# tenpy/cyten

Hardware: AMD Instinct MI355X
Metric: block-sparse tdot+SVD GFLOP/s (fp64) (higher is better)
Workload: dtype f64

## Files before the change

cyten_amd/csrc/jacobi_engine.hip:

```cpp
#include "jacobi_engine.h"

#include <algorithm>
#include <cmath>
#include <cstdlib>

namespace cyb {
constexpr double kPredictQuad = 16.0;
namespace {

typedef double d4 __attribute__((ext_vector_type(4)));
typedef double d2 __attribute__((ext_vector_type(2)));
#define GLOBAL_AS __attribute__((address_space(1)))
typedef const GLOBAL_AS d2* gc2;
typedef const GLOBAL_AS d2* gcp2;
typedef GLOBAL_AS double* gp;

constexpr int GS = JP + 2;
constexpr int QS = JP + 16;
constexpr int GK = 64;
constexpr int XS = GK + 2;
constexpr int NT = 256;
constexpr int NPAIR = JP / 2;
static_assert(JP == 32, "the wave tiling below assumes 32 x 32 pair problems");

// ... 844 lines not shown
            for (int e = lane; e < (CJ / 2) * CJ * 2; e += 64) {
                const int which = e / ((CJ / 2) * CJ), f = e % ((CJ / 2) * CJ);
                const int k = f / CJ, row = f % CJ;
                int p, q;
                pair_of(r, k, p, q);
                double* Xr = which ? Ur : Hr;
                double* Xi = which ? Ui : Hi;
                const double c = rot[k * 4], sn = rot[k * 4 + 1], fr = rot[k * 4 + 2], fi = -rot[k * 4 + 3];
                const double pr_ = Xr[row * CS + p], pi_ = Xi[row * CS + p], qr_ = Xr[row * CS + q], qi_ = Xi[row * CS + q];
                const double tr = fr * qr_ - fi * qi_, ti = fr * qi_ + fi * qr_;
                Xr[row * CS + p] = c * pr_ - sn * tr;
                Xi[row * CS + p] = c * pi_ - sn * ti;
                Xr[row * CS + q] = sn * pr_ + c * tr;
                Xi[row * CS + q] = sn * pi_ + c * ti;
            }
            __builtin_amdgcn_fence(__ATOMIC_RELEASE, "wavefront");
            __builtin_amdgcn_wave_barrier();
        }
    for (int e = lane; e < CJ * CJ; e += 64) {
        const int a = e / CJ, b = e % CJ;
        const double x = Ur[a * CS + b], y = Ui[a * CS + b];
        Vout[(2 * a) * VS + 2 * b] = x;
        Vout[(2 * a) * VS + 2 * b + 1] = -y;
        Vout[(2 * a + 1) * VS + 2 * b] = y;
        Vout[(2 * a + 1) * VS + 2 * b + 1] = x;
    }
    if (lane < CJ) {
        const double lam = Hr[lane * CS + lane];
        Gdiag[(2 * lane) * GS + 2 * lane] = lam;
        Gdiag[(2 * lane + 1) * GS + 2 * lane + 1] = lam;
    }
}

struct SScratch {
    double* gpart;
    unsigned int* ticket;
    unsigned int* ready;
    unsigned int* err;
    const int2* wgmap;
    const int2* wgent;
    unsigned long long* stamps;
    int stamp_round;
    int n_sweeps, n_mats;
    unsigned int* arrive;
    int* nsw;
    unsigned int* readyJ;
    int defer_j;
    int cross_every, cross_min_nb;
};
constexpr int SW_MAX_ENT = 64;

constexpr int SW_UN = 8;
constexpr int SW_PRE = 6;
constexpr int SWEEP_XREG = (4 * JP * GS > JP * GS + 2 * JP * VS) ? 4 * JP * GS : JP * GS + 2 * JP * VS;
constexpr int SWEEP_LDS_DOUBLES = JP * GS + SWEEP_XREG + 2 * JP * QS + 8;
constexpr size_t SWEEP_LDS_BYTES = 88 * 1024;
static_assert((size_t)SWEEP_LDS_DOUBLES * 8 + 1024 <= SWEEP_LDS_BYTES, "LDS request of the sweep kernel");
constexpr int SWEEP_WG_PER_CU = 1;

typedef unsigned int u32x2 __attribute__((ext_vector_type(2)));
union Q8 {
    u32x2 u;
    double d;
};

template <int SLEEP = 1>
__device__ __forceinline__ bool spin_until(const unsigned int* word, unsigned int target, unsigned int* err)
{
    const unsigned long long t0 = wall_clock64();
    unsigned int it = 0;
    while (__hip_atomic_load(word, __ATOMIC_RELAXED, __HIP_MEMORY_SCOPE_AGENT) < target) {
        __builtin_amdgcn_s_sleep(SLEEP);
        if ((++it & 63u) == 0u) {
            if (__hip_atomic_load(err, __ATOMIC_RELAXED, __HIP_MEMORY_SCOPE_AGENT) != 0u) return false;
            if (wall_clock64() - t0 > 100000000ull) {
                __hip_atomic_store(err, 1u, __ATOMIC_RELAXED, __HIP_MEMORY_SCOPE_AGENT);
                return false;
            }
        }
    }
    return true;
}

__device__ __forceinline__ void sweep_update_j(const __amdgpu_buffer_rsrc_t rsJ, const double* Qm, int P, int Q, int nvp, int j_begin,
                                               int nJ, int wave, int lane)
{
    const int un = lane & 15, ukq = lane >> 4;
    const double* ap0 = Qm + (lane >> 4) * QS + (lane & 15);
    const double* ap1 = ap0 + 16;
    double a0[JP / 4], a1[JP / 4];
#pragma unroll
    for (int kk = 0; kk < JP / 4; ++kk) {
        a0[kk] = ap0[kk * 4 * QS];
        a1[kk] = ap1[kk * 4 * QS];
    }
    auto off_of = [&](int c, int k) { return (unsigned int)(((int64_t)xrow(k, P, Q) * nvp + (j_begin + c) * 64 + wave * 16 + un) * 8); };
    auto load = [&](double (&x)[JP / 4], int c) {
#pragma unroll
        for (int kk = 0; kk < JP / 4; ++kk) {
            Q8 q;
            q.u = __builtin_amdgcn_raw_buffer_load_b64(rsJ, off_of(c, 4 * kk + ukq), 0, 16);
            x[kk] = q.d;
        }
    };
    double xb[JP / 4], xn[JP / 4];
    if (nJ > 0) load(xb, 0);
    for (int c = 0; c < nJ; ++c) {
        if (c + 1 < nJ) load(xn, c + 1);
        d4 acc[2] = {d4{0.0, 0.0, 0.0, 0.0}, d4{0.0, 0.0, 0.0, 0.0}};
#pragma unroll
        for (int kk = 0; kk < JP / 4; ++kk) {
            acc[0] = __builtin_amdgcn_mfma_f64_16x16x4f64(a0[kk], xb[kk], acc[0], 0, 0, 0);
            acc[1] = __builtin_amdgcn_mfma_f64_16x16x4f64(a1[kk], xb[kk], acc[1], 0, 0, 0);
        }
#pragma unroll
        for (int i = 0; i < 2; ++i)
#pragma unroll
            for (int q = 0; q < 4; ++q) {
                Q8 v;
                v.d = acc[i][q];
                __builtin_amdgcn_raw_buffer_store_b64(v.u, rsJ, off_of(c, i * 16 + (lane >> 4) + 4 * q), 0, 16);
            }
#pragma unroll
        for (int kk = 0; kk < JP / 4; ++kk) xb[kk] = xn[kk];
    }
}

template <bool CPLX>
__global__ void __launch_bounds__(NT, 1)
jacobi_sweep_kernel(const RPair* __restrict__ pairs, int max_inner, unsigned long long* __restrict__ offmax_bits, SScratch sc)
{
    extern __shared__ __attribute__((aligned(16))) double rsm[];
    double* Gs = rsm;
    double* G2 = Gs + JP * GS;
    double* Va = G2 + JP * GS;
    double* Vb = Va + JP * VS;
    double* Xc = G2;
    double* Qs0 = G2 + SWEEP_XREG;
    double* Qs1 = Qs0 + JP * QS;
    double* red = Qs1 + JP * QS;
    int* ibase = reinterpret_cast<int*>(red + 8);
    int* perm = ibase;
    int* zrow = ibase + JP;
    int* zout = ibase + 2 * JP;
    int* flags = ibase + 3 * JP;
    int* edone = flags + 4;

    const int tid = threadIdx.x;
    const int lane = tid & 63, wave = tid >> 6;
    const int2 went = sc.wgent ? sc.wgent[blockIdx.x] : make_int2((int)blockIdx.x, (int)blockIdx.x + 1);
    int max_rounds = 0;
    for (int e = went.x; e < went.y; ++e) max_rounds = max(max_rounds, pairs[sc.wgmap[e].x].nb - 1);
    const int n_sw = sc.n_sweeps;
    const bool one_entry = went.y - went.x == 1;
    int pendP = -1, pendQ = -1, pend_ground = 0;
    if (n_sw > 1) {
        if (tid < SW_MAX_ENT) edone[tid] = 0;
        __syncthreads();
    }
    for (int sw = 0; sw < n_sw; ++sw) {
    for (int round = 0; round < max_rounds; ++round)
    for (int ent = went.x; ent < went.y; ++ent) {
    const int2 wm = sc.wgmap[ent];
    const int pi = wm.x, part = wm.y;
    const RPair mt = pairs[pi];
    if (round >= mt.nb - 1) continue;
    if (n_sw > 1 && edone[ent - went.x]) continue;
    const int ground = sw * (mt.nb - 1) + round;
    const int G = mt.pad[0];
    unsigned int* ready = sc.ready + mt.pad[1];
    unsigned int* readyJ = sc.readyJ + mt.pad[1];
    unsigned int* ticket = sc.ticket + pi;
    double* Qs = (ground & 1) ? Qs1 : Qs0;
    const unsigned int pbytes = JP * JP * 8;
    const __amdgpu_buffer_rsrc_t rsW = __builtin_amdgcn_make_buffer_rsrc(mt.W, 0, (int)((size_t)mt.nvp * mt.lenp * 8), 0x00020000);
    const __amdgpu_buffer_rsrc_t rsJ =
        __builtin_amdgcn_make_buffer_rsrc(mt.J ? mt.J : mt.W, 0, mt.J ? (int)((size_t)mt.nvp * mt.nvp * 8) : 0, 0x00020000);
    const int cw = mt.lenp / 64, cj = mt.J ? mt.nvp / 64 : 0;
    const int w_begin = (int)((int64_t)part * cw / G), w_end = (int)((int64_t)(part + 1) * cw / G);
    const int j_begin = (int)((int64_t)part * cj / G), j_end = (int)((int64_t)(part + 1) * cj / G);
    const int nW = w_end - w_begin, nJ = j_end - j_begin;
    const bool defer = sc.defer_j && one_entry && G > 1 && nJ > 0 && round < mt.nb - 2;
    const int ct = defer ? nW : nW + nJ;
    const int pre_limit = (sc.defer_j && G > 1) ? min(ct, nW) : ct;
    const int un = lane & 15, ukq = lane >> 4;
#define SWEEP_STAMP(k)                                                                                            \
    do {                                                                                                          \
        if (sc.stamps && tid == 0 && round == sc.stamp_round) sc.stamps[(size_t)blockIdx.x * 8 + (k)] = wall_clock64(); \
    } while (0)

    {
        int P, Q;
        circle_pair(mt.nb, round, mt.slot, P, Q);
        if (P > Q) {
            const int t = P;
            P = Q;
            Q = t;
        }
        SWEEP_STAMP(0);
        __syncthreads();
        if (ground > 0) {
            if (tid == 0) {
                bool ok = spin_until(ready + (size_t)P * G + part, (unsigned int)ground, sc.err);
                ok = ok && spin_until(ready + (size_t)Q * G + part, (unsigned int)ground, sc.err);
                flags[1] = ok ? 1 : 0;
            }
            __syncthreads();
            if (!flags[1]) return;
        }
        SWEEP_STAMP(1);
        auto chunk_off = [&](int c, int k, bool& in_w) -> unsigned int {
            in_w = c < nW;
            const int ld = in_w ? mt.lenp : mt.nvp;
            const int cc = in_w ? w_begin + c : j_begin + (c - nW);
            return (unsigned int)(((int64_t)xrow(k, P, Q) * ld + cc * 64 + wave * 16 + un) * 8);
        };
        auto chunk_load = [&](int c, int k) -> double {
            bool in_w;
            const unsigned int off = chunk_off(c, k, in_w);
            Q8 q;
            q.u = in_w ? __builtin_amdgcn_raw_buffer_load_b64(rsW, off, 0, 16) : __builtin_amdgcn_raw_buffer_load_b64(rsJ, off, 0, 16);
            return q.d;
        };
        double xpre[SW_PRE][JP / 4];
        {
            const int ld = mt.lenp;
            d4 acc00 = d4{0.0, 0.0, 0.0, 0.0}, acc01 = acc00, acc11 = acc00;
            const int r = lane & 15, g2 = 2 * (lane >> 4);
            const unsigned int o0 = (unsigned int)(((int64_t)xrow(r, P, Q) * ld + g2) * 8);
            const unsigned int o1 = (unsigned int)(((int64_t)xrow(r + 16, P, Q) * ld + g2) * 8);
            const int c_begin = 8 * w_begin, c_end = 8 * w_end;
            constexpr int UN = SW_UN;
            d2 x0[UN], x1[UN], n0[UN], n1[UN];
            auto load = [&](d2 (&a0)[UN], d2 (&a1)[UN], int c0) {
#pragma unroll
                for (int u = 0; u < UN; ++u) {
                    const int c = min(c0 + 4 * u, c_end - 1);
                    Q16 qa, qb;
                    qa.u = __builtin_amdgcn_raw_buffer_load_b128(rsW, o0 + (unsigned int)c * 64u, 0, 16);
                    qb.u = __builtin_amdgcn_raw_buffer_load_b128(rsW, o1 + (unsigned int)c * 64u, 0, 16);
                    a0[u] = qa.d;
                    a1[u] = qb.d;
                }
            };
            if (c_begin + wave < c_end) load(x0, x1, c_begin + wave);
#pragma unroll
            for (int c = 0; c < SW_PRE; ++c) {
                if (c < pre_limit) {
#pragma unroll
                    for (int kk = 0; kk < JP / 4; ++kk) xpre[c][kk] = chunk_load(c, 4 * kk + ukq);
                }
            }
            for (int c0 = c_begin + wave; c0 < c_end; c0 += 4 * UN) {
                const bool more = c0 + 4 * UN < c_end;
                if (more) load(n0, n1, c0 + 4 * UN);
#pragma unroll
                for (int u = 0; u < UN; ++u) {
                    if (c0 + 4 * u < c_end) {
                        acc00 = __builtin_amdgcn_mfma_f64_16x16x4f64(x0[u].x, x0[u].x, acc00, 0, 0, 0);
                        acc01 = __builtin_amdgcn_mfma_f64_16x16x4f64(x0[u].x, x1[u].x, acc01, 0, 0, 0);
                        acc11 = __builtin_amdgcn_mfma_f64_16x16x4f64(x1[u].x, x1[u].x, acc11, 0, 0, 0);
                        acc00 = __builtin_amdgcn_mfma_f64_16x16x4f64(x0[u].y, x0[u].y, acc00, 0, 0, 0);
                        acc01 = __builtin_amdgcn_mfma_f64_16x16x4f64(x0[u].y, x1[u].y, acc01, 0, 0, 0);
                        acc11 = __builtin_amdgcn_mfma_f64_16x16x4f64(x1[u].y, x1[u].y, acc11, 0, 0, 0);
                    }
                }
                if (more) {
#pragma unroll
                    for (int u = 0; u < UN; ++u) {
                        x0[u] = n0[u];
                        x1[u] = n1[u];
                    }
                }
            }
            double* wpart = Xc + wave * (JP * GS);
#pragma unroll
            for (int q = 0; q < 4; ++q) {
                const int rr = (lane >> 4) + 4 * q, cc = lane & 15;
                wpart[rr * GS + cc] = acc00[q];
                wpart[rr * GS + 16 + cc] = acc01[q];
                wpart[(16 + cc) * GS + rr] = acc01[q];
                wpart[(16 + rr) * GS + 16 + cc] = acc11[q];
            }
        }
        __syncthreads();
        SWEEP_STAMP(2);
        {
            const int gi = tid >> 3, gj = 4 * (tid & 7);
            d2 lo = d2{0.0, 0.0}, hi = d2{0.0, 0.0};
#pragma unroll
            for (int w = 0; w < 4; ++w) {
                const double* src = Xc + w * (JP * GS) + gi * GS + gj;
                lo.x += src[0];
                lo.y += src[1];
                hi.x += src[2];
                hi.y += src[3];
            }
            if (G > 1) {
                const __amdgpu_buffer_rsrc_t rs_all = __builtin_amdgcn_make_buffer_rsrc(
                    sc.gpart + ((size_t)pi * 2 + (size_t)(ground & 1)) * RGMAX * (JP * JP), 0, (int)(pbytes * G), 0x00020000);
                Q16 a, b;
                a.d = lo;
                b.d = hi;
                const unsigned int off = (unsigned int)part * pbytes + (unsigned int)tid * 32u;
                __builtin_amdgcn_raw_buffer_store_b128(a.u, rs_all, off, 0, 16);
                __builtin_amdgcn_raw_buffer_store_b128(b.u, rs_all, off + 16u, 0, 16);
                asm volatile("s_waitcnt vmcnt(0)" ::: "memory");
                __syncthreads();
                if (tid == 0) __hip_atomic_fetch_add(ticket, 1u, __ATOMIC_RELAXED, __HIP_MEMORY_SCOPE_AGENT);
                if (pendP >= 0) {
                    if (tid == 0) {
                        bool ok = spin_until(readyJ + (size_t)pendP * G + part, (unsigned int)pend_ground, sc.err);
                        ok = ok && spin_until(readyJ + (size_t)pendQ * G + part, (unsigned int)pend_ground, sc.err);
                        flags[1] = ok ? 1 : 0;
                    }
                    __syncthreads();
                    if (!flags[1]) return;
                    sweep_update_j(rsJ, (pend_ground & 1) ? Qs1 : Qs0, pendP, pendQ, mt.nvp, j_begin, nJ, wave, lane);
                    asm volatile("s_waitcnt vmcnt(0)" ::: "memory");
                    __syncthreads();
                    if (tid == 0) {
                        __hip_atomic_store(readyJ + (size_t)pendP * G + part, (unsigned int)(pend_ground + 1), __ATOMIC_RELAXED, __HIP_MEMORY_SCOPE_AGENT);
                        __hip_atomic_store(readyJ + (size_t)pendQ * G + part, (unsigned int)(pend_ground + 1), __ATOMIC_RELAXED, __HIP_MEMORY_SCOPE_AGENT);
                    }
                    pendP = -1;
                }
                if (tid == 0) flags[1] = spin_until(ticket, (unsigned int)G * (unsigned int)(ground + 1), sc.err) ? 1 : 0;
                __syncthreads();
                if (!flags[1]) return;
                lo = d2{0.0, 0.0};
                hi = d2{0.0, 0.0};
                for (int g0 = 0; g0 < G; g0 += 4) {
                    Q16 pa[4], pb[4];
#pragma unroll
                    for (int g = 0; g < 4; ++g) {
                        if (g0 + g < G) {
                            pa[g].u = __builtin_amdgcn_raw_buffer_load_b128(rs_all, (unsigned int)(g0 + g) * pbytes + (unsigned int)tid * 32u, 0, 16);
                            pb[g].u = __builtin_amdgcn_raw_buffer_load_b128(rs_all, (unsigned int)(g0 + g) * pbytes + (unsigned int)tid * 32u + 16u, 0, 16);
                        }
                    }
#pragma unroll
                    for (int g = 0; g < 4; ++g) {
                        if (g0 + g < G) {
                            lo += pa[g].d;
                            hi += pb[g].d;
                        }
                    }
                }
            }
            double* dst = Gs + gi * GS + gj;
            dst[0] = lo.x;
            dst[1] = lo.y;
            dst[2] = hi.x;
            dst[3] = hi.y;
        }
        __syncthreads();
        SWEEP_STAMP(3);
        if (tid == 0) flags[0] = 0;
        __syncthreads();
        if (tid < JP) {
            double g = Gs[tid * GS + tid];
            if constexpr (CPLX) g = fmax(g, Gs[(tid ^ 1) * GS + (tid ^ 1)]);
            const int z = (g > 0.0 && g <= mt.thr2) ? 1 : 0;
            zrow[tid] = z;
            perm[tid] = tid;
            if (z) flags[0] = 1;
        }
        __syncthreads();
        const bool any_null = flags[0] != 0;
        if (any_null) {
            for (int e = tid; e < JP * JP; e += NT) {
                const int i = e / JP, j = e % JP;
                if (zrow[i] || zrow[j]) Gs[i * GS + j] = 0.0;
            }
            __syncthreads();
        }
        const double off = gram_offmax(Gs, red, tid);
        if (part == 0 && tid == 0) atomicMax(offmax_bits + (size_t)sw * sc.n_mats + mt.mat, (unsigned long long)__double_as_longlong(off));
        const bool skip = off <= mt.tol && !any_null;
        if (!skip) {
            double* Ga = Gs;
            double* Gb = G2;
            double* Vc = Va;
            double* Vn = Vb;
            bool pos_is_interleaved = false;
            const int cross_k = sc.cross_every > 0 ? sc.cross_every : max(4, (mt.nb + 2) / 4);
            const bool cross = sc.cross_every != 0 && !any_null && mt.nb >= sc.cross_min_nb && (round % cross_k) != 0;
            if constexpr (CPLX) {
                if (tid < 64) hermitian_pivot_solve(Gs, G2, Vb, Va, Gs, max_inner, tid, 0.25 * mt.tol * mt.tol, cross);
                __syncthreads();
            } else {
            auto cpos = [](int i) { return i < JB ? 2 * i : 2 * (i - JB) + 1; };
            pos_is_interleaved = cross;
            if (cross) {
                for (int e = tid; e < JP * JP; e += NT) {
                    const int i = e / JP, j = e % JP;
                    Gb[cpos(i) * GS + cpos(j)] = Ga[i * GS + j];
// ... 3 lines not shown
                Ga = Gb;
                Gb = t;
            } else
                for (int e = tid; e < JP * VS; e += NT) Va[e] = ((e / VS) == (e % VS)) ? 1.0 : 0.0;
            __syncthreads();
            {
                const int pr = tid >> 4, pc = tid & 15;
                const int r0 = 2 * pr, c0 = 2 * pc;
                const int dr0 = cross ? r0 : ring_next(r0), dr1 = cross ? ((r0 + 3) & (JP - 1)) : ring_next(r0 + 1);
                const int dc0 = cross ? c0 : ring_next(c0), dc1 = cross ? ((c0 + 3) & (JP - 1)) : ring_next(c0 + 1);
                const int n_steps = cross ? JB : JP - 1;
                for (int sweep = 0; sweep < (off <= mt.tol ? 0 : max_inner); ++sweep) {
                    for (int r = 0; r < n_steps; ++r) {
                        const d2 g0 = *reinterpret_cast<const d2*>(Ga + r0 * GS + c0);
                        const d2 g1 = *reinterpret_cast<const d2*>(Ga + (r0 + 1) * GS + c0);
                        const d2 ac = *reinterpret_cast<const d2*>(Ga + c0 * GS + c0);
                        const double dc = Ga[(c0 + 1) * GS + c0 + 1];
                        const d2 v0 = *reinterpret_cast<const d2*>(Vc + r0 * VS + c0);
                        const d2 v1 = *reinterpret_cast<const d2*>(Vc + (r0 + 1) * VS + c0);
                        double c1, s1, c2, s2;
                        jacobi_rot_bf(ac.x, dc, ac.y, c2, s2, 0.25 * mt.tol * mt.tol);
                        const int rsrc = (lane & 48) | pr;
                        c1 = __shfl(c2, rsrc);
                        s1 = __shfl(s2, rsrc);
                        const double hik = c1 * g0.x - s1 * g1.x, hil = c1 * g0.y - s1 * g1.y;
                        const double hjk = s1 * g0.x + c1 * g1.x, hjl = s1 * g0.y + c1 * g1.y;
                        double nik = c2 * hik - s2 * hil, nil = s2 * hik + c2 * hil;
                        double njk = c2 * hjk - s2 * hjl, njl = s2 * hjk + c2 * hjl;
                        if (pr == pc) {
                            nil = 0.0;
                            njk = 0.0;
                        }
                        Gb[dr0 * GS + dc0] = nik;
                        Gb[dr0 * GS + dc1] = nil;
                        Gb[dr1 * GS + dc0] = njk;
                        Gb[dr1 * GS + dc1] = njl;
                        Vn[r0 * VS + dc0] = c2 * v0.x - s2 * v0.y;
                        Vn[r0 * VS + dc1] = s2 * v0.x + c2 * v0.y;
                        Vn[(r0 + 1) * VS + dc0] = c2 * v1.x - s2 * v1.y;
                        Vn[(r0 + 1) * VS + dc1] = s2 * v1.x + c2 * v1.y;
                        __syncthreads();
                        double* t = Ga;
                        Ga = Gb;
                        Gb = t;
                        t = Vc;
                        Vc = Vn;
                        Vn = t;
                    }
                    if (sweep + 1 < max_inner) {
                        const double off_in = gram_offmax(Ga, red, tid);
                        if (off_in <= 0.25 * mt.tol) break;
                    }
                }
            }
            }
            __syncthreads();
            SWEEP_STAMP(4);
            if (off > mt.tol && tid < 64) {
                const int li = lane & (JP - 1);
                const int li_idx = pos_is_interleaved ? ((li & 1) ? JB + (li >> 1) : (li >> 1)) : li;
                const double g = xrow(li_idx, P, Q) < mt.nv ? Ga[li * GS + li] : -1.0e300;
                const int glo = __double2loint(g), ghi = __double2hiint(g);
                int rk = 0;
#pragma unroll
                for (int j = 0; j < JP; ++j) {
                    const double gj = __hiloint2double(__builtin_amdgcn_readlane(ghi, j), __builtin_amdgcn_readlane(glo, j));
                    rk += (gj > g || (gj == g && j < li)) ? 1 : 0;
                }
                if (lane < JP) perm[rk] = lane;
            }
            __syncthreads();
            for (int e = tid; e < JP * JP; e += NT) {
                const int k = e / JP, m = e % JP;
                Qs[k * QS + m] = Vc[k * VS + perm[m]];
            }
            if (tid < JP) {
                const int pp = perm[tid];
                zout[tid] = zrow[pos_is_interleaved ? ((pp & 1) ? JB + (pp >> 1) : (pp >> 1)) : pp];
            }
            __syncthreads();
            SWEEP_STAMP(5);
            if (ct > nW) {
                if (tid == 0) {
                    bool ok = spin_until(readyJ + (size_t)P * G + part, (unsigned int)ground, sc.err);
                    ok = ok && spin_until(readyJ + (size_t)Q * G + part, (unsigned int)ground, sc.err);
                    flags[1] = ok ? 1 : 0;
                }
                __syncthreads();
                if (!flags[1]) return;
#pragma unroll
                for (int c = 0; c < SW_PRE; ++c) {
                    if (c >= pre_limit && c < ct) {
#pragma unroll
                        for (int kk = 0; kk < JP / 4; ++kk) xpre[c][kk] = chunk_load(c, 4 * kk + ukq);
                    }
                }
            }
            if (ct > 0) {
                const double* ap0 = Qs + (lane >> 4) * QS + (lane & 15);
                const double* ap1 = ap0 + 16;
                double a0[JP / 4], a1[JP / 4];
#pragma unroll
                for (int kk = 0; kk < JP / 4; ++kk) {
                    a0[kk] = ap0[kk * 4 * QS];
                    a1[kk] = ap1[kk * 4 * QS];
                }
                int zr[2][4];
#pragma unroll
                for (int i = 0; i < 2; ++i)
#pragma unroll
                    for (int q = 0; q < 4; ++q) zr[i][q] = zout[i * 16 + (lane >> 4) + 4 * q];
                auto apply = [&](int c, const double (&xb)[JP / 4]) {
                    d4 acc[2] = {d4{0.0, 0.0, 0.0, 0.0}, d4{0.0, 0.0, 0.0, 0.0}};
#pragma unroll
                    for (int kk = 0; kk < JP / 4; ++kk) {
                        acc[0] = __builtin_amdgcn_mfma_f64_16x16x4f64(a0[kk], xb[kk], acc[0], 0, 0, 0);
                        acc[1] = __builtin_amdgcn_mfma_f64_16x16x4f64(a1[kk], xb[kk], acc[1], 0, 0, 0);
                    }
                    const bool zero_null = c < nW;
#pragma unroll
                    for (int i = 0; i < 2; ++i)
#pragma unroll
                        for (int q = 0; q < 4; ++q) {
                            const int row = i * 16 + (lane >> 4) + 4 * q;
                            bool in_w;
                            const unsigned int o = chunk_off(c, row, in_w);
                            Q8 v;
                            v.d = (zero_null && zr[i][q]) ? 0.0 : acc[i][q];
                            if (in_w) __builtin_amdgcn_raw_buffer_store_b64(v.u, rsW, o, 0, 16);
                            else __builtin_amdgcn_raw_buffer_store_b64(v.u, rsJ, o, 0, 16);
                        }
                };
#pragma unroll
                for (int c = 0; c < SW_PRE; ++c)
                    if (c < ct) apply(c, xpre[c]);
                if (ct > SW_PRE) {
                    double xb[JP / 4], xn[JP / 4];
#pragma unroll
                    for (int kk = 0; kk < JP / 4; ++kk) xb[kk] = chunk_load(SW_PRE, 4 * kk + ukq);
                    for (int c = SW_PRE; c < ct; ++c) {
                        if (c + 1 < ct) {
#pragma unroll
                            for (int kk = 0; kk < JP / 4; ++kk) xn[kk] = chunk_load(c + 1, 4 * kk + ukq);
                        }
                        apply(c, xb);
#pragma unroll
                        for (int kk = 0; kk < JP / 4; ++kk) xb[kk] = xn[kk];
                    }
                }
            }
        }
        if (defer && !skip) {
            pendP = P;
            pendQ = Q;
            pend_ground = ground;
        }
        asm volatile("s_waitcnt vmcnt(0)" ::: "memory");
        __syncthreads();
        if (tid == 0) {
            if (skip && nJ > 0) {
                (void)spin_until(readyJ + (size_t)P * G + part, (unsigned int)ground, sc.err);
                (void)spin_until(readyJ + (size_t)Q * G + part, (unsigned int)ground, sc.err);
            }
            __hip_atomic_store(ready + (size_t)P * G + part, (unsigned int)(ground + 1), __ATOMIC_RELAXED, __HIP_MEMORY_SCOPE_AGENT);
            __hip_atomic_store(ready + (size_t)Q * G + part, (unsigned int)(ground + 1), __ATOMIC_RELAXED, __HIP_MEMORY_SCOPE_AGENT);
            if (!(defer && !skip)) {
                __hip_atomic_store(readyJ + (size_t)P * G + part, (unsigned int)(ground + 1), __ATOMIC_RELAXED, __HIP_MEMORY_SCOPE_AGENT);
                __hip_atomic_store(readyJ + (size_t)Q * G + part, (unsigned int)(ground + 1), __ATOMIC_RELAXED, __HIP_MEMORY_SCOPE_AGENT);
            }
            if (n_sw > 1 && round == mt.nb - 2) __hip_atomic_fetch_add(sc.arrive + mt.mat, 1u, __ATOMIC_RELAXED, __HIP_MEMORY_SCOPE_AGENT);
        }
        SWEEP_STAMP(6);
    }
    }
    if (n_sw == 1) break;
    __syncthreads();
    if (tid == 0) {
        int all = 1, ok = 1;
        for (int ent = went.x; ent < went.y && ok; ++ent) {
            if (edone[ent - went.x]) continue;
            const int2 wm = sc.wgmap[ent];
            const RPair mt = pairs[wm.x];
            const unsigned int entries = (unsigned int)(mt.nb / 2) * (unsigned int)mt.pad[0];
            if (!spin_until<32>(sc.arrive + mt.mat, entries * (unsigned int)(sw + 1), sc.err)) {
                ok = 0;
                break;
            }
            const double off = __longlong_as_double((long long)__hip_atomic_load(offmax_bits + (size_t)sw * sc.n_mats + mt.mat, __ATOMIC_RELAXED, __HIP_MEMORY_SCOPE_AGENT));
            const double prev = sw ? __longlong_as_double((long long)__hip_atomic_load(offmax_bits + (size_t)(sw - 1) * sc.n_mats + mt.mat,
                                                                                      __ATOMIC_RELAXED, __HIP_MEMORY_SCOPE_AGENT))
                                   : 1e300;
            const bool stagnated = sw + 1 >= 6 && off <= 64.0 * mt.tol && off >= 0.5 * prev;
            const bool predicted = off <= 0.1 * sqrt(mt.tol) && prev < 1.0 && off <= prev * sqrt(prev) && off <= kPredictQuad * prev * prev;
            if (off <= mt.tol || stagnated || predicted) {
                edone[ent - went.x] = 1;
                if (mt.slot == 0 && wm.y == 0) sc.nsw[mt.mat] = sw + 1;
            } else all = 0;
        }
        flags[1] = ok;
        flags[2] = all;
    }
    __syncthreads();
    if (!flags[1] || flags[2]) return;
    }
#undef SWEEP_STAMP
}

}

int jacobi_orthogonalise(cyb_ctx_t ctx, const std::vector<JMat>& h_mats, int max_sweeps,
                         std::vector<int32_t>& sweeps_out, bool cplx)
{
    const int n = (int)h_mats.size();
    sweeps_out.assign((size_t)n, 0);
    if (n == 0) return CYB_OK;
    hipStream_t st = ctx->stream;

    std::vector<int> active;
    for (int i = 0; i < n; ++i) {
        if (h_mats[(size_t)i].nv <= 1) sweeps_out[(size_t)i] = 0;
        else active.push_back(i);
    }
    static const bool one_launch_ok = getenv("CYB_JACOBI_PERSWEEP") == nullptr && getenv("CYB_JACOBI_TRACE") == nullptr &&
                                      getenv("CYB_JACOBI_STAMPS") == nullptr && getenv("CYB_JACOBI_NOPREDICT") == nullptr;
    static const bool one_launch_all = getenv("CYB_JACOBI_ONELAUNCH") != nullptr;
    int nb_max_all = 0;
    for (int i = 0; i < n; ++i) nb_max_all = std::max(nb_max_all, h_mats[(size_t)i].nb);
    const int n_sw_dev = (one_launch_ok && (one_launch_all || nb_max_all <= 16)) ? max_sweeps : 1;
    const size_t w_off = (size_t)n * (size_t)n_sw_dev;
    const size_t b_off = (sizeof(unsigned long long) * w_off + 2 * sizeof(unsigned int) * (size_t)n + 15) / 16 * 16;
    std::vector<unsigned long long> h_off(b_off / 8 + 2);
    bool one_launch_done = false;
    std::vector<int> cached_order, cached_G;
    uint64_t cached_at = 0;
    void* cached_img = nullptr;
    size_t cached_map_off = 0;
    std::vector<double> prev_off((size_t)n, 1e300);
    int status = CYB_OK;
    for (int sweep = 1; sweep <= max_sweeps && !active.empty(); ++sweep) {
        std::vector<int> order = active;
        std::stable_sort(order.begin(), order.end(),
                         [&](int a, int b) { return h_mats[(size_t)a].nb > h_mats[(size_t)b].nb; });
        std::vector<JWork> wl;
        int max_nb = 0;
        for (int m : order) {
// ... 104 lines not shown
            size_t used = np;
            while (true) {
                int best = -1;
                double worst = 0.0;
                for (int m : order) {
                    const JMat& jm = h_mats[(size_t)m];
                    const int cw_ = jm.lenp / 64;
                    if (Gm[(size_t)m] >= RGMAX || Gm[(size_t)m] >= cw_ || used + (size_t)jm.nb / 2 > sweep_slots) continue;
                    const double c = chain(m);
                    if (c > worst) {
                        worst = c;
                        best = m;
                    }
                }
                if (best < 0) break;
                ++Gm[(size_t)best];
                used += (size_t)h_mats[(size_t)best].nb / 2;
            }
            if (g_env > 0)
                for (int m : order) Gm[(size_t)m] = std::max(1, std::min({g_env, RGMAX, h_mats[(size_t)m].lenp / 64}));
            size_t total = 0;
            for (int m : order) total += (size_t)h_mats[(size_t)m].nb / 2 * (size_t)Gm[(size_t)m];
            if (total <= sweep_slots || (!no_share && total == np)) {
                std::vector<int> flag_base((size_t)n, 0);
                int fb = (int)np;
                for (int m : order) {
                    flag_base[(size_t)m] = fb;
                    fb += h_mats[(size_t)m].nb * Gm[(size_t)m];
                }
                std::vector<int2> wgmap;
                for (size_t k = 0; k < np; ++k) {
                    rp[k].pad[0] = Gm[(size_t)wl[k].mat];
                    rp[k].pad[1] = flag_base[(size_t)wl[k].mat];
                    for (int g = 0; g < Gm[(size_t)wl[k].mat]; ++g) wgmap.push_back(make_int2((int)k, g));
                }
                std::vector<int2> wgent;
                if (wgmap.size() > sweep_slots) {
                    std::vector<size_t> ent_before;
                    size_t acc = 0;
                    for (int m : order) {
                        ent_before.push_back(acc);
                        acc += (size_t)h_mats[(size_t)m].nb / 2;
                    }
                    ent_before.push_back(acc);
                    size_t best_i = 0, best_m = 0;
                    double best_cost = 1e300;
                    for (size_t i = 0; i <= order.size(); ++i) {
                        const size_t D = ent_before[i], S = acc - D;
                        if (D > sweep_slots || (S > 0 && D >= sweep_slots)) break;
                        const size_t m = S ? (S + (sweep_slots - D) - 1) / (sweep_slots - D) : 1;
                        const double own = (double)(h_mats[(size_t)order[0]].nb - 1);
                        const double shared = i < order.size() ? (double)m * (double)(h_mats[(size_t)order[i]].nb - 1) : 0.0;
                        const double cost = std::max(own, shared);
                        if (cost < best_cost) {
                            best_cost = cost;
                            best_i = i;
                            best_m = m;
                        }
                    }
                    const size_t D = ent_before[best_i];
                    for (size_t e = 0; e < D; ++e) wgent.push_back(make_int2((int)e, (int)e + 1));
                    for (size_t e = D; e < wgmap.size(); e += best_m)
                        wgent.push_back(make_int2((int)e, (int)std::min(e + best_m, wgmap.size())));
                }
                const size_t n_wg = wgent.empty() ? wgmap.size() : wgent.size();
                std::vector<int> g_now;
                for (int m : order) g_now.push_back(Gm[(size_t)m]);
                const size_t map_off = (sizeof(RPair) * np + 255) / 256 * 256;
                const size_t ent_off = (map_off + sizeof(int2) * wgmap.size() + 255) / 256 * 256;
                if (!(cached_img && order == cached_order && g_now == cached_G && ctx->n_uploads - cached_at < (uint64_t)cyb_ctx_s::kSlots / 2 - 1)) {
                    std::vector<char> img(ent_off + sizeof(int2) * wgent.size());
                    memcpy(img.data(), rp.data(), sizeof(RPair) * np);
                    memcpy(img.data() + map_off, wgmap.data(), sizeof(int2) * wgmap.size());
                    if (!wgent.empty()) memcpy(img.data() + ent_off, wgent.data(), sizeof(int2) * wgent.size());
                    status = ctx->upload(img.data(), img.size(), &cached_img);
                    if (status != CYB_OK) break;
                    cached_order = order;
                    cached_G = g_now;
                    cached_at = ctx->n_uploads;
                    cached_map_off = map_off;
                }
                void* d_rp2 = cached_img;
                void* d_map = static_cast<char*>(cached_img) + cached_map_off;
                static bool attr2_set = false;
                if (!attr2_set) {
                    if (hipFuncSetAttribute(reinterpret_cast<const void*>(jacobi_sweep_kernel<false>), hipFuncAttributeMaxDynamicSharedMemorySize,
                                            (int)SWEEP_LDS_BYTES) != hipSuccess ||
                        hipFuncSetAttribute(reinterpret_cast<const void*>(jacobi_sweep_kernel<true>), hipFuncAttributeMaxDynamicSharedMemorySize,
                                            (int)SWEEP_LDS_BYTES) != hipSuccess) {
                        set_error("jacobi: cannot reserve %zu bytes of LDS for the sweep kernel", SWEEP_LDS_BYTES);
                        status = CYB_ERR_HIP;
                        break;
                    }
                    attr2_set = true;
                }
                SScratch ss;
                ss.gpart = rs.gpart;
                ss.ticket = d_ready;
                ss.ready = d_ready;
                ss.readyJ = d_ready + n_ready;
                static const bool no_defer_j = getenv("CYB_JACOBI_NODEFERJ") != nullptr;
                ss.defer_j = no_defer_j ? 0 : 1;
                static const int cross_env = getenv("CYB_JACOBI_CROSS") ? atoi(getenv("CYB_JACOBI_CROSS")) : -1;
                static const bool cross_small = getenv("CYB_JACOBI_CROSS_SMALL") != nullptr;
                ss.cross_every = (max_inner == 1 || cross_small) ? cross_env : 0;
                static const int cross_min_nb = getenv("CYB_JACOBI_CROSS_MINNB") ? atoi(getenv("CYB_JACOBI_CROSS_MINNB")) : 0;
                ss.cross_min_nb = cross_min_nb;
                ss.err = rs.err;
                ss.wgmap = static_cast<const int2*>(d_map);
                ss.wgent = wgent.empty() ? nullptr : reinterpret_cast<const int2*>(static_cast<char*>(cached_img) + ent_off);
                ss.stamps = wgent.empty() ? rs.stamps : nullptr;
                ss.stamp_round = std::min(3, max_nb - 2);
                size_t max_ent = 1;
                for (const int2& we : wgent) max_ent = std::max(max_ent, (size_t)(we.y - we.x));
                const bool one_launch = n_sw_dev > 1 && sweep == 1 && max_ent <= (size_t)SW_MAX_ENT;
                ss.n_sweeps = one_launch ? n_sw_dev : 1;
                ss.n_mats = n;
                ss.arrive = reinterpret_cast<unsigned int*>(d_off + w_off);
                ss.nsw = reinterpret_cast<int*>(ss.arrive + n);
                one_launch_done = one_launch;
                if (cplx)
                    hipLaunchKernelGGL(jacobi_sweep_kernel<true>, dim3((unsigned)n_wg), dim3(NT), SWEEP_LDS_BYTES, st,
                                       static_cast<const RPair*>(d_rp2), max_inner, d_off, ss);
                else
                    hipLaunchKernelGGL(jacobi_sweep_kernel<false>, dim3((unsigned)n_wg), dim3(NT), SWEEP_LDS_BYTES, st,
                                       static_cast<const RPair*>(d_rp2), max_inner, d_off, ss);
                if (ss.stamps && wgmap.size() <= 2048) {
                    std::vector<unsigned long long> hs(8 * wgmap.size());
                    if (hipMemcpyAsync(hs.data(), rs.stamps, sizeof(unsigned long long) * hs.size(), hipMemcpyDeviceToHost, st) == hipSuccess &&
                        hipStreamSynchronize(st) == hipSuccess) {
                        double acc[6] = {0, 0, 0, 0, 0, 0};
                        int cntw = 0;
                        const int mbig = order.front();
                        for (size_t b = 0; b < wgmap.size(); ++b) {
                            if (wl[(size_t)wgmap[b].x].mat != mbig) continue;
                            for (int k = 0; k < 6; ++k) acc[k] += (double)(hs[8 * b + k + 1] - hs[8 * b + k]) * 0.01;
                            ++cntw;
                        }
                        if (cntw)
                            fprintf(stderr, "[jacobi sweep stamps] sweep %d round %d, largest matrix (G=%d, %d workgroups of %zu): wait %.2f load+gram %.2f "
                                            "exch %.2f defl+eig %.2f sort %.2f upd+publish %.2f us\n",
                                    sweep, ss.stamp_round, Gm[(size_t)mbig], cntw, wgmap.size(), acc[0] / cntw, acc[1] / cntw,
                                    acc[2] / cntw, acc[3] / cntw, acc[4] / cntw, acc[5] / cntw);
                    }
                }
                did_sweep = true;
            }
        }
        if (!did_sweep && cplx) {
            set_error("block-Jacobi on embedded complex rows needs the persistent sweep kernel (list too large for one launch)");
            status = CYB_ERR_UNSUPPORTED;
            break;
        }
        if (!did_sweep) {
        cached_img = nullptr;
        {
            void* d_mats_v = nullptr;
            status = ctx->upload(h_mats.data(), sizeof(JMat) * (size_t)n, &d_mats_v);
            if (status == CYB_OK) status = ctx->upload(wl.data(), sizeof(JWork) * wl.size(), &d_wl);
            if (status == CYB_OK) status = ctx->upload(rp.data(), sizeof(RPair) * np, &d_rp);
            if (status != CYB_OK) break;
            d_mats = static_cast<const JMat*>(d_mats_v);
            if (hipMemsetAsync(sc.cnt, 0, b_c, st) != hipSuccess) {
                status = CYB_ERR_HIP;
                break;
            }
        }
        int pend_round = -1;
        size_t pend_cnt = 0;
        auto flush_pending = [&]() {
            if (pend_round < 0) return;
            const int U = (int)std::min<size_t>(16, std::max<size_t>(1, (size_t)(3 * ctx->n_cu) / pend_cnt));
            hipLaunchKernelGGL(jacobi_update_kernel, dim3((unsigned)(pend_cnt * U)), dim3(NT), 0, st, d_mats,
                               static_cast<const JWork*>(d_wl), pend_round, U, sc, pend_round & 1, 0, 1);
            pend_round = -1;
        };
        for (int r = 0; r < max_nb - 1; ++r) {
            size_t cnt = 0;
            for (int m : order) {
                if (h_mats[(size_t)m].nb - 1 > r) cnt += (size_t)h_mats[(size_t)m].nb / 2;
                else break;
            }
            if (cnt == 0) break;
            const bool fused = !legacy && cnt <= (size_t)fused_max && cnt <= (size_t)ctx->n_cu;
            if (fused) {
                flush_pending();
                int G = (int)std::min<size_t>(kGmax, (size_t)ctx->n_cu / cnt);
                if (g_env > 0 && (size_t)g_env * cnt <= (size_t)ctx->n_cu) G = std::min(g_env, kGmax);
                G = std::max(G, 1);
                hipLaunchKernelGGL(jacobi_round_kernel, dim3((unsigned)(cnt * G)), dim3(NT), ROUND_LDS_BYTES, st,
                                   static_cast<const RPair*>(d_rp), r, G, max_inner, d_off, rs);
                if (rs.stamps && r == max_nb / 2 && cnt * (size_t)G <= 2048) {
                    std::vector<unsigned long long> hs(8 * cnt * G);
                    if (hipMemcpyAsync(hs.data(), rs.stamps, sizeof(unsigned long long) * hs.size(), hipMemcpyDeviceToHost, st) == hipSuccess &&
                        hipStreamSynchronize(st) == hipSuccess) {
                        double acc[6] = {0, 0, 0, 0, 0, 0}, tot = 0, mx = 0;
                        for (size_t b = 0; b < cnt * G; ++b) {
                            for (int k = 0; k < 6; ++k) acc[k] += (double)(hs[8 * b + k + 1] - hs[8 * b + k]) * 0.01;
                            const double t = (double)(hs[8 * b + 6] - hs[8 * b]) * 0.01;
                            tot += t;
                            mx = std::max(mx, t);
                        }
                        const double nb_ = (double)(cnt * G);
                        fprintf(stderr, "[jacobi stamps] sweep %d round %d: %zu pairs x G=%d | gram %.2f exch %.2f defl %.2f eig %.2f sort %.2f upd %.2f | wg mean %.2f max %.2f us\n",
                                sweep, r, cnt, G, acc[0] / nb_, acc[1] / nb_, acc[2] / nb_, acc[3] / nb_, acc[4] / nb_, acc[5] / nb_, tot / nb_, mx);
                    }
                }
                continue;
            }
// ... 81 lines not shown
```

Baseline: 5561.

## Reorder sweep kernel waits and loads to overlap prefetch with cross-workgroup exchange

After: 5749, median of 6. +3.4%, better.

```diff
diff --git a/cyten_amd/csrc/jacobi_engine.hip b/cyten_amd/csrc/jacobi_engine.hip
--- a/cyten_amd/csrc/jacobi_engine.hip
+++ b/cyten_amd/csrc/jacobi_engine.hip
@@ -950,6 +950,32 @@
     return true;
 }
 
+template <int SLEEP = 1>
+__device__ __forceinline__ bool spin_until2(const unsigned int* word0, const unsigned int* word1, unsigned int target, unsigned int* err)
+{
+    const unsigned long long t0 = wall_clock64();
+    unsigned int it = 0;
+    for (;;) {
+        const unsigned int v0 = __hip_atomic_load(word0, __ATOMIC_RELAXED, __HIP_MEMORY_SCOPE_AGENT);
+        const unsigned int v1 = __hip_atomic_load(word1, __ATOMIC_RELAXED, __HIP_MEMORY_SCOPE_AGENT);
+        if ((v0 >= target) & (v1 >= target)) return true;
+        __builtin_amdgcn_s_sleep(SLEEP);
+        if ((++it & 63u) == 0u) {
+            if (__hip_atomic_load(err, __ATOMIC_RELAXED, __HIP_MEMORY_SCOPE_AGENT) != 0u) return false;
+            if (wall_clock64() - t0 > 100000000ull) {
+                __hip_atomic_store(err, 1u, __ATOMIC_RELAXED, __HIP_MEMORY_SCOPE_AGENT);
+                return false;
+            }
+        }
+    }
+}
+template <bool RORD>
+__device__ __forceinline__ bool spin_pair(const unsigned int* word0, const unsigned int* word1, unsigned int target, unsigned int* err)
+{
+    if constexpr (RORD) return spin_until2(word0, word1, target, err);
+    else return spin_until(word0, target, err) && spin_until(word1, target, err);
+}
+
 __device__ __forceinline__ void sweep_update_j(const __amdgpu_buffer_rsrc_t rsJ, const double* Qm, int P, int Q, int nvp, int j_begin,
                                                int nJ, int wave, int lane)
 {
@@ -994,7 +1020,7 @@
     }
 }
 
-template <bool CPLX>
+template <bool CPLX, bool RORD>
 __global__ void __launch_bounds__(NT, 1)
 jacobi_sweep_kernel(const RPair* __restrict__ pairs, int max_inner, unsigned long long* __restrict__ offmax_bits, SScratch sc)
 {
@@ -1069,9 +1095,7 @@
         __syncthreads();
         if (ground > 0) {
             if (tid == 0) {
-                bool ok = spin_until(ready + (size_t)P * G + part, (unsigned int)ground, sc.err);
-                ok = ok && spin_until(ready + (size_t)Q * G + part, (unsigned int)ground, sc.err);
-                flags[1] = ok ? 1 : 0;
+                flags[1] = spin_pair<RORD>(ready + (size_t)P * G + part, ready + (size_t)Q * G + part, (unsigned int)ground, sc.err) ? 1 : 0;
             }
             __syncthreads();
             if (!flags[1]) return;
@@ -1091,6 +1115,15 @@
             return q.d;
         };
         double xpre[SW_PRE][JP / 4];
+        auto issue_xpre = [&]() {
+#pragma unroll
+            for (int c = 0; c < SW_PRE; ++c) {
+                if (c < pre_limit) {
+#pragma unroll
+                    for (int kk = 0; kk < JP / 4; ++kk) xpre[c][kk] = chunk_load(c, 4 * kk + ukq);
+                }
+            }
+        };
         {
             const int ld = mt.lenp;
             d4 acc00 = d4{0.0, 0.0, 0.0, 0.0}, acc01 = acc00, acc11 = acc00;
@@ -1111,28 +1144,49 @@
                     a1[u] = qb.d;
                 }
             };
+            auto gram = [&](const d2 (&a0)[UN], const d2 (&a1)[UN], int c0) {
+#pragma unroll
+                for (int u = 0; u < UN; ++u) {
+                    if (c0 + 4 * u < c_end) {
+                        acc00 = __builtin_amdgcn_mfma_f64_16x16x4f64(a0[u].x, a0[u].x, acc00, 0, 0, 0);
+                        acc01 = __builtin_amdgcn_mfma_f64_16x16x4f64(a0[u].x, a1[u].x, acc01, 0, 0, 0);
+                        acc11 = __builtin_amdgcn_mfma_f64_16x16x4f64(a1[u].x, a1[u].x, acc11, 0, 0, 0);
+                        acc00 = __builtin_amdgcn_mfma_f64_16x16x4f64(a0[u].y, a0[u].y, acc00, 0, 0, 0);
+                        acc01 = __builtin_amdgcn_mfma_f64_16x16x4f64(a0[u].y, a1[u].y, acc01, 0, 0, 0);
+                        acc11 = __builtin_amdgcn_mfma_f64_16x16x4f64(a1[u].y, a1[u].y, acc11, 0, 0, 0);
+                    }
+                }
+            };
+            if constexpr (RORD) {
+                int c0 = c_begin + wave;
+                if (c0 < c_end) {
+                    load(x0, x1, c0);
+                    for (;;) {
+                        if (c0 + 4 * UN < c_end) {
+                            load(n0, n1, c0 + 4 * UN);
+                            gram(x0, x1, c0);
+                        } else {
+                            gram(x0, x1, c0);
+                            break;
+                        }
+                        c0 += 4 * UN;
+                        if (c0 + 4 * UN < c_end) {
+                            load(x0, x1, c0 + 4 * UN);
+                            gram(n0, n1, c0);
+                        } else {
+                            gram(n0, n1, c0);
+                            break;
+                        }
+                        c0 += 4 * UN;
+                    }
+                }
+            } else {
             if (c_begin + wave < c_end) load(x0, x1, c_begin + wave);
-#pragma unroll
-            for (int c = 0; c < SW_PRE; ++c) {
-                if (c < pre_limit) {
-#pragma unroll
-                    for (int kk = 0; kk < JP / 4; ++kk) xpre[c][kk] = chunk_load(c, 4 * kk + ukq);
-                }
-            }
+            issue_xpre();
             for (int c0 = c_begin + wave; c0 < c_end; c0 += 4 * UN) {
                 const bool more = c0 + 4 * UN < c_end;
                 if (more) load(n0, n1, c0 + 4 * UN);
-#pragma unroll
-                for (int u = 0; u < UN; ++u) {
-                    if (c0 + 4 * u < c_end) {
-                        acc00 = __builtin_amdgcn_mfma_f64_16x16x4f64(x0[u].x, x0[u].x, acc00, 0, 0, 0);
-                        acc01 = __builtin_amdgcn_mfma_f64_16x16x4f64(x0[u].x, x1[u].x, acc01, 0, 0, 0);
-                        acc11 = __builtin_amdgcn_mfma_f64_16x16x4f64(x1[u].x, x1[u].x, acc11, 0, 0, 0);
-                        acc00 = __builtin_amdgcn_mfma_f64_16x16x4f64(x0[u].y, x0[u].y, acc00, 0, 0, 0);
-                        acc01 = __builtin_amdgcn_mfma_f64_16x16x4f64(x0[u].y, x1[u].y, acc01, 0, 0, 0);
-                        acc11 = __builtin_amdgcn_mfma_f64_16x16x4f64(x1[u].y, x1[u].y, acc11, 0, 0, 0);
-                    }
-                }
+                gram(x0, x1, c0);
                 if (more) {
 #pragma unroll
                     for (int u = 0; u < UN; ++u) {
@@ -1140,6 +1194,7 @@
                         x1[u] = n1[u];
                     }
                 }
+            }
             }
             double* wpart = Xc + wave * (JP * GS);
 #pragma unroll
@@ -1153,6 +1208,7 @@
         }
         __syncthreads();
         SWEEP_STAMP(2);
+        if constexpr (RORD) __builtin_amdgcn_s_waitcnt(0x0F70);
         {
             const int gi = tid >> 3, gj = 4 * (tid & 7);
             d2 lo = d2{0.0, 0.0}, hi = d2{0.0, 0.0};
@@ -1164,9 +1220,9 @@
                 hi.x += src[2];
                 hi.y += src[3];
             }
+            const __amdgpu_buffer_rsrc_t rs_all = __builtin_amdgcn_make_buffer_rsrc(
+                sc.gpart + ((size_t)pi * 2 + (size_t)(ground & 1)) * RGMAX * (JP * JP), 0, (int)(pbytes * G), 0x00020000);
             if (G > 1) {
-                const __amdgpu_buffer_rsrc_t rs_all = __builtin_amdgcn_make_buffer_rsrc(
-                    sc.gpart + ((size_t)pi * 2 + (size_t)(ground & 1)) * RGMAX * (JP * JP), 0, (int)(pbytes * G), 0x00020000);
                 Q16 a, b;
                 a.d = lo;
                 b.d = hi;
@@ -1176,11 +1232,12 @@
                 asm volatile("s_waitcnt vmcnt(0)" ::: "memory");
                 __syncthreads();
                 if (tid == 0) __hip_atomic_fetch_add(ticket, 1u, __ATOMIC_RELAXED, __HIP_MEMORY_SCOPE_AGENT);
+            }
+            if constexpr (RORD) issue_xpre();
+            if (G > 1) {
                 if (pendP >= 0) {
                     if (tid == 0) {
-                        bool ok = spin_until(readyJ + (size_t)pendP * G + part, (unsigned int)pend_ground, sc.err);
-                        ok = ok && spin_until(readyJ + (size_t)pendQ * G + part, (unsigned int)pend_ground, sc.err);
-                        flags[1] = ok ? 1 : 0;
+                        flags[1] = spin_pair<RORD>(readyJ + (size_t)pendP * G + part, readyJ + (size_t)pendQ * G + part, (unsigned int)pend_ground, sc.err) ? 1 : 0;
                     }
                     __syncthreads();
                     if (!flags[1]) return;
@@ -1350,9 +1407,7 @@
             SWEEP_STAMP(5);
             if (ct > nW) {
                 if (tid == 0) {
-                    bool ok = spin_until(readyJ + (size_t)P * G + part, (unsigned int)ground, sc.err);
-                    ok = ok && spin_until(readyJ + (size_t)Q * G + part, (unsigned int)ground, sc.err);
-                    flags[1] = ok ? 1 : 0;
+                    flags[1] = spin_pair<RORD>(readyJ + (size_t)P * G + part, readyJ + (size_t)Q * G + part, (unsigned int)ground, sc.err) ? 1 : 0;
                 }
                 __syncthreads();
                 if (!flags[1]) return;
@@ -1406,6 +1461,30 @@
                     double xb[JP / 4], xn[JP / 4];
 #pragma unroll
                     for (int kk = 0; kk < JP / 4; ++kk) xb[kk] = chunk_load(SW_PRE, 4 * kk + ukq);
+                    if constexpr (RORD) {
+                        auto fetch = [&](double (&x)[JP / 4], int c) {
+#pragma unroll
+                            for (int kk = 0; kk < JP / 4; ++kk) x[kk] = chunk_load(c, 4 * kk + ukq);
+                        };
+                        for (int c = SW_PRE;;) {
+                            if (c + 1 < ct) {
+                                fetch(xn, c + 1);
+                                apply(c, xb);
+                            } else {
+                                apply(c, xb);
+                                break;
+                            }
+                            ++c;
+                            if (c + 1 < ct) {
+                                fetch(xb, c + 1);
+                                apply(c, xn);
+                            } else {
+                                apply(c, xn);
+                                break;
+                            }
+                            ++c;
+                        }
+                    } else
                     for (int c = SW_PRE; c < ct; ++c) {
                         if (c + 1 < ct) {
 #pragma unroll
@@ -1427,8 +1506,11 @@
         __syncthreads();
         if (tid == 0) {
             if (skip && nJ > 0) {
-                (void)spin_until(readyJ + (size_t)P * G + part, (unsigned int)ground, sc.err);
-                (void)spin_until(readyJ + (size_t)Q * G + part, (unsigned int)ground, sc.err);
+                if constexpr (RORD) (void)spin_until2(readyJ + (size_t)P * G + part, readyJ + (size_t)Q * G + part, (unsigned int)ground, sc.err);
+                else {
+                    (void)spin_until(readyJ + (size_t)P * G + part, (unsigned int)ground, sc.err);
+                    (void)spin_until(readyJ + (size_t)Q * G + part, (unsigned int)ground, sc.err);
+                }
             }
             __hip_atomic_store(ready + (size_t)P * G + part, (unsigned int)(ground + 1), __ATOMIC_RELAXED, __HIP_MEMORY_SCOPE_AGENT);
             __hip_atomic_store(ready + (size_t)Q * G + part, (unsigned int)(ground + 1), __ATOMIC_RELAXED, __HIP_MEMORY_SCOPE_AGENT);
@@ -1699,11 +1781,15 @@
                 }
                 void* d_rp2 = cached_img;
                 void* d_map = static_cast<char*>(cached_img) + cached_map_off;
+                static const bool round_order = !(getenv("CYB_JACOBI_ROUND_ORDER") && atoi(getenv("CYB_JACOBI_ROUND_ORDER")) == 0);
+                typedef void (*sweep_fn_t)(const RPair*, int, unsigned long long*, SScratch);
+                static const sweep_fn_t sweep_fn[2] = {round_order ? jacobi_sweep_kernel<false, true> : jacobi_sweep_kernel<false, false>,
+                                                       round_order ? jacobi_sweep_kernel<true, true> : jacobi_sweep_kernel<true, false>};
                 static bool attr2_set = false;
                 if (!attr2_set) {
-                    if (hipFuncSetAttribute(reinterpret_cast<const void*>(jacobi_sweep_kernel<false>), hipFuncAttributeMaxDynamicSharedMemorySize,
+                    if (hipFuncSetAttribute(reinterpret_cast<const void*>(sweep_fn[0]), hipFuncAttributeMaxDynamicSharedMemorySize,
                                             (int)SWEEP_LDS_BYTES) != hipSuccess ||
-                        hipFuncSetAttribute(reinterpret_cast<const void*>(jacobi_sweep_kernel<true>), hipFuncAttributeMaxDynamicSharedMemorySize,
+                        hipFuncSetAttribute(reinterpret_cast<const void*>(sweep_fn[1]), hipFuncAttributeMaxDynamicSharedMemorySize,
                                             (int)SWEEP_LDS_BYTES) != hipSuccess) {
                         set_error("jacobi: cannot reserve %zu bytes of LDS for the sweep kernel", SWEEP_LDS_BYTES);
                         status = CYB_ERR_HIP;
@@ -1736,12 +1822,8 @@
                 ss.arrive = reinterpret_cast<unsigned int*>(d_off + w_off);
                 ss.nsw = reinterpret_cast<int*>(ss.arrive + n);
                 one_launch_done = one_launch;
-                if (cplx)
-                    hipLaunchKernelGGL(jacobi_sweep_kernel<true>, dim3((unsigned)n_wg), dim3(NT), SWEEP_LDS_BYTES, st,
-                                       static_cast<const RPair*>(d_rp2), max_inner, d_off, ss);
-                else
-                    hipLaunchKernelGGL(jacobi_sweep_kernel<false>, dim3((unsigned)n_wg), dim3(NT), SWEEP_LDS_BYTES, st,
-                                       static_cast<const RPair*>(d_rp2), max_inner, d_off, ss);
+                hipLaunchKernelGGL(sweep_fn[cplx ? 1 : 0], dim3((unsigned)n_wg), dim3(NT), SWEEP_LDS_BYTES, st,
+                                   static_cast<const RPair*>(d_rp2), max_inner, d_off, ss);
                 if (ss.stamps && wgmap.size() <= 2048) {
                     std::vector<unsigned long long> hs(8 * wgmap.size());
                     if (hipMemcpyAsync(hs.data(), rs.stamps, sizeof(unsigned long long) * hs.size(), hipMemcpyDeviceToHost, st) == hipSuccess &&
```
